# myfavouritekk/vdetlib

Measured on AMD Instinct MI355X. Metric: boxes/sec whole-node (NMS+temporal-conv+link), 300f×10k-box synth; mAP parity, higher is better.
Workload: dtype f32; 1 GPU; configs[1]+[2]: 1 video/GPU, 300 frames x 10000 boxes x 200 classes; per-(frame,class) NMS thresh 0.30 + temporal max-pool w=3 + 3-tap temporal convolution; greedy tubelets: 10 tracks/class (stop < 0.90), IoU-link >= 0.50, spatial max-pool IoU > 0.70 + completion + temporal max-pool; frames=300, boxes=10000, classes=200, scores=rand, parallelism=video-per-gpu x1, 4 distinct videos in flight per GPU

## Files before the change

### include/vdet_hip.h

```cpp
#ifndef VDET_HIP_H
#define VDET_HIP_H

#include <stdint.h>

#ifdef __cplusplus
extern "C" {
#endif

typedef struct vdet_ctx vdet_ctx;

typedef enum vdet_status {
    VDET_OK = 0,
    VDET_EINVAL = -1,
    VDET_ECAP = -2,
    VDET_EHIP = -3,
    VDET_EDIVZERO = -4,
    VDET_ENOMEM = -5,
    VDET_EINDEX = -6,
    VDET_EAGAIN = -7
} vdet_status;


int vdet_create(vdet_ctx **out, int device);
int vdet_destroy(vdet_ctx *ctx);
// ... 67 lines not shown
                        int class0, int use_score_thresh, float score_thresh, int topk, double nms_thresh,
                        float *d_dets, int32_t *d_sel_idx, int32_t *d_det_cnt, int32_t *d_keep, int32_t *d_keep_cnt);

int vdet_nms_volume_ordered(vdet_ctx *ctx, const float *d_boxes, const uint16_t *d_order, const int32_t *d_ncand,
                            int64_t F, int64_t B, int64_t C, double thresh, int32_t *d_keep_idx,
                            int32_t *d_keep_cnt, int64_t cap);

int vdet_video_batch(vdet_ctx *ctx, const float *d_boxes, const float *d_scores, const int64_t *h_frame_off,
                     int64_t V, int64_t B, int64_t C, double nms_thres, double thres, int max_tracks,
                     double link_thres, int max_frames, float *d_tracks, float *d_anchors, int32_t *d_ntracks,
                     int64_t cap, int32_t *d_keep_idx, int32_t *d_keep_cnt, double overlap_thres, int window,
                     double *d_det_score, double *d_pooled, float *d_boxes_out);

int vdet_volume_pass_batch(vdet_ctx *ctx, const float *d_scores, const int64_t *h_frame_off, int64_t V, int64_t B,
                           int64_t C, int window, float pad_max, const float *h_taps, float bias, float pad_conv,
                           float *d_out_max, float *d_out_conv, int use_score_thresh, float score_thresh);

int vdet_argsort_volume(vdet_ctx *ctx, const float *d_scores, int layout, int64_t F, int64_t B, int64_t C,
                        int use_score_thresh, float score_thresh, uint16_t *d_order, int32_t *d_ncand);

int vdet_temporal_maxpool_f32(vdet_ctx *ctx, const float *d_in, float *d_out, int64_t F, int64_t S,
                              int window, float pad);

int vdet_temporal_conv_f32(vdet_ctx *ctx, const float *d_in, float *d_out, int64_t F, int64_t S,
                           const float *h_taps, int K, float bias, float pad);

int vdet_temporal_maxpool_conv_f32(vdet_ctx *ctx, const float *d_in, float *d_out_max, float *d_out_conv, int64_t F,
                                   int64_t S, int window, float pad_max, const float *h_taps, float bias, float pad_conv);

int vdet_volume_pass(vdet_ctx *ctx, const float *d_scores, int64_t F, int64_t B, int64_t C, int window,
                     float pad_max, const float *h_taps, float bias, float pad_conv, float *d_out_max,
                     float *d_out_conv, int use_score_thresh, float score_thresh);

int vdet_track_volume(vdet_ctx *ctx, const float *d_boxes, const float *d_scores, int64_t F, int64_t B,
                      int64_t C, double nms_thres, double thres, int max_tracks, double link_thres,
                      int max_frames, float *d_tracks, float *d_anchors, int32_t *d_ntracks);

int vdet_nms_track_volume(vdet_ctx *ctx, const float *d_boxes, const float *d_scores, int64_t F, int64_t B,
                          int64_t C, double nms_thres, double thres, int max_tracks, double link_thres,
                          int max_frames, float *d_tracks, float *d_anchors, int32_t *d_ntracks, int64_t cap,
                          int32_t *d_keep_idx, int32_t *d_keep_cnt);

int vdet_rescore_tracks(vdet_ctx *ctx, const float *d_tracks, const int32_t *d_ntracks, const float *d_boxes,
                        const float *d_scores, int64_t F, int64_t B, int64_t C, int max_tracks,
                        double overlap_thres, int window, double *d_det_score, double *d_pooled,
                        float *d_boxes_out);

int vdet_eval_gt_upload(vdet_ctx *ctx, const int32_t *h_vid, const int64_t *h_frame, const int32_t *h_slot, const double *h_boxes,
                        int64_t G, const int64_t *h_vid_nf, int64_t NV, int K, double *d_gt_boxes, int32_t *d_gt_off,
                        int64_t *d_vid_meta);

int vdet_eval_match_tracks(vdet_ctx *ctx, const double *d_gt_boxes, const int32_t *d_gt_off, const int64_t *d_vid_meta, int K,
                           int rule, double iou_thr, int vid, int64_t F, int64_t C, int T, const float *d_boxes, int box_stride,
                           const void *d_scores, int scores_f64, const int32_t *d_ntracks, const int32_t *h_col_slot,
                           int32_t *d_st_slot, double *d_st_score, uint8_t *d_st_tp, int64_t st_len, int64_t st_cap,
                           int64_t *h_count);

int vdet_eval_match_tracks_batch(vdet_ctx *ctx, const double *d_gt_boxes, const int32_t *d_gt_off, const int64_t *d_vid_meta,
                                 int K, int rule, double iou_thr, const int32_t *h_vid, const int64_t *h_frame_off, int64_t V,
                                 int64_t C, int T, const float *d_boxes, int box_stride, const void *d_scores, int scores_f64,
                                 const int32_t *d_ntracks, const int32_t *h_col_slot, int32_t *d_st_slot, double *d_st_score,
                                 uint8_t *d_st_tp, int64_t st_len, int64_t st_cap, int64_t *h_count);

int vdet_eval_match_keep(vdet_ctx *ctx, const double *d_gt_boxes, const int32_t *d_gt_off, const int64_t *d_vid_meta, int K,
                         int rule, double iou_thr, int vid, const float *d_boxes, const float *d_scores, int layout, int64_t F,
                         int64_t B, int64_t C, const int32_t *d_keep_idx, const int32_t *d_keep_cnt, int64_t cap,
// ... 199 lines not shown
```

### vdetlib_amd/_lib.py

```python
import ctypes
import importlib.util
import os
import threading

_HERE = os.path.dirname(os.path.abspath(__file__))
LIB_PATH = os.path.join(_HERE, "libvdet_hip.so")

VDET_OK, VDET_EINVAL, VDET_ECAP, VDET_EHIP, VDET_EDIVZERO, VDET_ENOMEM, VDET_EINDEX, VDET_EAGAIN = 0, -1, -2, -3, -4, -5, -6, -7
LAYOUT_FBC, LAYOUT_FCB = 0, 1

_i64, _f64, _f32, _vp, _ci = ctypes.c_int64, ctypes.c_double, ctypes.c_float, ctypes.c_void_p, ctypes.c_int
SYMBOLS = {
    "vdet_create": (_ci, [ctypes.POINTER(_vp), _ci]),
    "vdet_destroy": (_ci, [_vp]),
    "vdet_set_stream": (_ci, [_vp, _vp]),
    "vdet_reset_stream": (_ci, [_vp]),
    "vdet_sync": (_ci, [_vp]),
    "vdet_last_error": (ctypes.c_char_p, [_vp]),
    "vdet_version": (ctypes.c_char_p, []),
    "vdet_last_timing_ms": (_ci, [_vp, _vp]),
    "vdet_last_launches": (_ci, [_vp, _vp]),
    "vdet_set_timing": (_ci, [_vp, _ci]),
    "vdet_query": (_ci, [_vp, _ci]),
    "vdet_set_cache": (_ci, [_vp, _ci]),
    "vdet_invalidate": (_ci, [_vp]),
    "vdet_set_async": (_ci, [_vp, _ci]),
    "vdet_nms_f32": (_ci, [_vp, _vp, _i64, _i64, _ci, _f64, _vp, _vp, ctypes.POINTER(_i64)]),
    "vdet_track_det_nms_f32": (_ci, [_vp, _vp, _i64, _i64, _vp, _i64, _i64, _f64, _vp, ctypes.POINTER(_i64)]),
    "vdet_track_det_nms_batch": (_ci, [_vp, _vp, _vp, _i64, _vp, _vp, _i64, _i64, _f64, _vp, _vp]),
    "vdet_iou_f64": (_ci, [_vp, _vp, _i64, _vp, _i64, _vp]),
    "vdet_svm_scores_f64": (_ci, [_vp, _vp, _i64, _i64, _vp, _vp, _i64, _vp]),
    "vdet_svm_scores_f32": (_ci, [_vp, _vp, _i64, _i64, _vp, _vp, _i64, _vp]),
    "vdet_spatial_maxpool_f64": (_ci, [_vp, _vp, _vp, _i64, _vp, _vp, _vp, _i64, _f64, _vp, _vp]),
    "vdet_series_completion_f64": (_ci, [_vp, _vp, _vp, _i64]),
    "vdet_series_maxpool_f64": (_ci, [_vp, _vp, _vp, _vp, _i64, _ci, _f64]),
    "vdet_series_interp_f64": (_ci, [_vp, _vp, _vp, _vp, _vp, _vp, _i64, _ci, _vp]),
    "vdet_threshold_topk": (_ci, [_vp, _vp, _ci, _i64, _i64, _ci, _ci, _f64, _ci, _vp, _vp]),
    "vdet_conv1d_f32": (_ci, [_vp, _vp, _ci, _ci, _vp, _vp, _ci, _ci, _ci, _vp]),
    "vdet_nms_volume": (_ci, [_vp, _vp, _vp, _ci, _i64, _i64, _i64, _f64, _ci, _f32, _vp, _vp, _i64]),
    "vdet_nms_volume_topk": (_ci, [_vp, _vp, _vp, _ci, _i64, _i64, _i64, _f64, _ci, _f32, _ci, _vp, _vp, _i64]),
    "vdet_det_nms_volume": (_ci, [_vp, _vp, _vp, _i64, _i64, _i64, _ci, _ci, _f32, _ci, _f64, _vp, _vp, _vp, _vp, _vp]),
    "vdet_nms_volume_ordered": (_ci, [_vp, _vp, _vp, _vp, _i64, _i64, _i64, _f64, _vp, _vp, _i64]),
    "vdet_argsort_volume": (_ci, [_vp, _vp, _ci, _i64, _i64, _i64, _ci, _f32, _vp, _vp]),
    "vdet_video_batch": (_ci, [_vp, _vp, _vp, _vp, _i64, _i64, _i64, _f64, _f64, _ci, _f64, _ci, _vp, _vp, _vp, _i64, _vp, _vp,
                               _f64, _ci, _vp, _vp, _vp]),
    "vdet_volume_pass_batch": (_ci, [_vp, _vp, _vp, _i64, _i64, _i64, _ci, _f32, _vp, _f32, _f32, _vp, _vp, _ci, _f32]),
    "vdet_volume_pass": (_ci, [_vp, _vp, _i64, _i64, _i64, _ci, _f32, _vp, _f32, _f32, _vp, _vp, _ci, _f32]),
    "vdet_track_volume": (_ci, [_vp, _vp, _vp, _i64, _i64, _i64, _f64, _f64, _ci, _f64, _ci, _vp, _vp, _vp]),
    "vdet_nms_track_volume": (_ci, [_vp, _vp, _vp, _i64, _i64, _i64, _f64, _f64, _ci, _f64, _ci, _vp, _vp, _vp,
                                    _i64, _vp, _vp]),
    "vdet_rescore_tracks": (_ci, [_vp, _vp, _vp, _vp, _vp, _i64, _i64, _i64, _ci, _f64, _ci, _vp, _vp, _vp]),
    "vdet_temporal_maxpool_f32": (_ci, [_vp, _vp, _vp, _i64, _i64, _ci, _f32]),
    "vdet_temporal_conv_f32": (_ci, [_vp, _vp, _vp, _i64, _i64, _vp, _ci, _f32, _f32]),
    "vdet_temporal_maxpool_conv_f32": (_ci, [_vp, _vp, _vp, _vp, _i64, _i64, _ci, _f32, _vp, _f32, _f32]),
    "vdet_eval_gt_upload": (_ci, [_vp, _vp, _vp, _vp, _vp, _i64, _vp, _i64, _ci, _vp, _vp, _vp]),
    "vdet_eval_match_tracks": (_ci, [_vp, _vp, _vp, _vp, _ci, _ci, _f64, _ci, _i64, _i64, _ci, _vp, _ci, _vp, _ci, _vp, _vp,
                                     _vp, _vp, _vp, _i64, _i64, ctypes.POINTER(_i64)]),
    "vdet_eval_match_tracks_batch": (_ci, [_vp, _vp, _vp, _vp, _ci, _ci, _f64, _vp, _vp, _i64, _i64, _ci, _vp, _ci, _vp, _ci, _vp,
                                           _vp, _vp, _vp, _vp, _i64, _i64, ctypes.POINTER(_i64)]),
# ... 130 lines not shown
        if rc == VDET_OK:
            return
        msg = self.error()
        if rc == VDET_EDIVZERO:
            raise ZeroDivisionError("float division")
        if rc in (VDET_EINVAL, VDET_ECAP):
            raise ValueError(msg or "invalid argument")
        if rc == VDET_ENOMEM:
            raise MemoryError(msg)
        if rc == VDET_EINDEX:
            raise IndexError(msg or "list index out of range")
        if rc == VDET_EAGAIN:
            raise RetryError(msg)
        raise RuntimeError("libvdet_hip: %s (rc=%d)" % (msg, rc))

    def set_stream(self, stream_ptr):
        self.check(self.lib.vdet_set_stream(self.h, _vp(stream_ptr or 0)))

    def reset_stream(self):
        self.check(self.lib.vdet_reset_stream(self.h))

    def sync(self):
        self.check(self.lib.vdet_sync(self.h))

    def set_cache(self, on):
        self.check(self.lib.vdet_set_cache(self.h, 1 if on else 0))

    def invalidate(self):
        self.check(self.lib.vdet_invalidate(self.h))

    def set_async(self, on):
        self.check(self.lib.vdet_set_async(self.h, 1 if on else 0))

    def query(self, what):
        return int(self.lib.vdet_query(self.h, int(what)))

    def set_timing(self, on):
        self.check(self.lib.vdet_set_timing(self.h, int(on)))

    def last_timing(self):
        ms = (ctypes.c_float * 16)()
        n = (ctypes.c_int * 16)()
        self.check(self.lib.vdet_last_timing_ms(self.h, ms))
        self.check(self.lib.vdet_last_launches(self.h, n))
        names = ["iou_bits", "adj_build", "sort", "walk", "temporal", "merge_sort", "iou_bits_general", "other",
                 "transpose_keys", "track_pick", "track_link", "track_suppress", "rescore_spatial", "rescore_series",
                 "sort_fallback", "track_loop"]
        return {k: (float(ms[i]), int(n[i])) for i, k in enumerate(names)}


def get_context(device=-1):
    with _lock:
        c = _ctxs.get(device)
        if c is None:
            c = Context(device)
            _ctxs[device] = c
        return c
```

### vdetlib_amd/csrc/temporal_kernels.hpp

```cpp
#pragma once
#include <hip/hip_runtime.h>
#include <stdint.h>

#include "nms_kernels.hpp"

namespace vdet {

struct Taps { float w[32]; };

__device__ __forceinline__ bool seg_in(const int2 *__restrict__ seg, int64_t f, int64_t g, int64_t F)
{
    if (!seg) return g >= 0 && g < F;
    const int2 r = seg[f];
    return g >= (int64_t)r.x && g < (int64_t)r.y;
}

__device__ __forceinline__ float4 splat4(float v) { return make_float4(v, v, v, v); }

struct MaxAcc {
    float4 m; uint32_t nan;
    __device__ __forceinline__ void init(float4 v)
    {
        m = v;
        nan = (v.x != v.x) | ((v.y != v.y) << 1) | ((v.z != v.z) << 2) | ((v.w != v.w) << 3);
// ... 224 lines not shown
            const float4 s = win[i][H];
            uint4 k4 = make_uint4(score_key(s.x), score_key(s.y), score_key(s.z), score_key(s.w));
            if (use_thr) {
                if (!(s.x > thr)) k4.x = 0u;
                if (!(s.y > thr)) k4.y = 0u;
                if (!(s.z > thr)) k4.z = 0u;
                if (!(s.w > thr)) k4.w = 0u;
            }
            tb[loff[i]] = k4.x; tb[loff[i] + TB] = k4.y; tb[loff[i] + 2 * TB] = k4.z; tb[loff[i] + 3 * TB] = k4.w;
        }
        __syncthreads();
        uint32_t *kf = keys + (int64_t)f * C4 * 4 * B + b0;
        const bool vec_ok = (B & 3) == 0;
#pragma unroll
        for (int i = 0; i < ITEMS; ++i) {
            const int idx = tid + NT * i;
            const int cc = idx >> (tb_shift - 2), q = idx & qmask;
            if (cc < C4 * 4 && 4 * q < rows) {
                const uint4 k4 = *reinterpret_cast<const uint4 *>(tb + cc * TB + ((4 * q) ^ (((cc >> 2) & qmask) << 2)));
                const int o = cc * B + 4 * q;
                if (vec_ok && 4 * q + 3 < rows) {
                    vp_store_u4(reinterpret_cast<uint4 *>(kf + o), k4);
                } else {
                    kf[o] = k4.x;
                    if (4 * q + 1 < rows) kf[o + 1] = k4.y;
                    if (4 * q + 2 < rows) kf[o + 2] = k4.z;
                    if (4 * q + 3 < rows) kf[o + 3] = k4.w;
                }
            }
        }
    }
}

template <int MODE>
__global__ __launch_bounds__(256) void temporal_scalar_kernel(const float *__restrict__ in, float *__restrict__ out,
                                                              int64_t F, int64_t S, int W, float pad, float bias,
                                                              Taps taps, const int2 *__restrict__ seg)
{
    const int64_t i = (int64_t)blockIdx.x * 256 + threadIdx.x;
    if (i >= F * S) return;
    const int64_t f = i / S, s = i - f * S;
    const int H = W / 2;
    if (MODE == 0) {
        float m = 0.0f;
        bool nan = false;
        for (int k = 0; k < W; ++k) {
            const int64_t g = f + k - H;
            const int64_t gc = min(max(g, (int64_t)0), F - 1);
            float v = in[gc * S + s];
            v = (g == gc && seg_in(seg, f, g, F)) ? v : pad;
            nan |= (v != v);
            m = (k == 0) ? v : fmaxf(m, v);
        }
        out[i] = nan ? __uint_as_float(0x7FC00000u) : m;
    } else {
        float acc = bias;
        for (int k = 0; k < W; ++k) {
            const int64_t g = f + k - H;
            const int64_t gc = min(max(g, (int64_t)0), F - 1);
            float v = in[gc * S + s];
            v = (g == gc && seg_in(seg, f, g, F)) ? v : pad;
            acc = acc + taps.w[k] * v;
        }
        out[i] = acc;
    }
}
// ... 30 lines not shown
```

### vdetlib_amd/csrc/vdet_capi.hip

```cpp
#include <hip/hip_runtime.h>
#include <atomic>
#include <chrono>

#include <algorithm>
#include <cmath>
#include <cstdarg>
#include <cstdio>
#include <cstdlib>
#include <cstring>
#include <string>
#include <vector>

#include "../../include/vdet_hip.h"
#include "nms_kernels.hpp"
#include "binsort_kernels.hpp"
#include "small_kernels.hpp"
#include "detnms_kernels.hpp"
#include "fused_kernels.hpp"
#include "adjrows_kernels.hpp"
#include "graphlists_kernels.hpp"
#include "temporal_kernels.hpp"
#include "tubelet_kernels.hpp"
#include "track_kernels.hpp"
#include "batch_kernels.hpp"
// ... 59 lines not shown
{
    if (cnt->pool_used > cnt->pool_max) cnt->pool_max = cnt->pool_used;
}

struct StagedTab {
    DevBuf dev;
    std::vector<char> host;
    std::vector<char> key;
    bool valid = false;
    long long uploads = 0;
};

struct ListsKey {
    const void *scores = nullptr;
    int64_t C = 0;
    int layout = -1, use_thr = 0;
    float thr = 0;
    int topk = 0;
    bool operator==(const ListsKey &o) const { return scores == o.scores && C == o.C && layout == o.layout && use_thr == o.use_thr && (!use_thr || thr == o.thr) && topk == o.topk; }
};

struct NmsPlan {
    std::vector<GroupDesc> groups;
    std::vector<TileDesc> tiles;
    std::vector<TilePair> pairs;
    std::vector<std::pair<int, int>> batch_tiles;
    std::vector<std::pair<int, int>> batch_pairs;
    std::vector<ListItem> ditems;
    std::vector<std::pair<int, int>> batch_ditems;
    size_t bits_words_max = 0;
    int64_t ntot = 0;
    int nmax = 0;
};

}

struct vdet_ctx {
    int device = 0;
    hipStream_t stream = nullptr;
    hipStream_t own_stream = nullptr;
    std::string err;
    Counters *d_cnt = nullptr;
    int latched = 0;
    size_t bits_budget = (size_t)1 << 30;
    size_t max_lds = 160 * 1024;
    int n_cu = 256;
    DevBuf boxes, scores, keys, excl, frames, groups, tiles, bits, rowz, rowmeta, groupz, adj, comp, origidx,
        out64, trk_frames, trk_boxes, b1, b2, iou_out, order, ncand, keepidx, keepcnt, gflags, pairs, tkeys, tstate, visited, heads, xkeys, xord, wmeta, wmeta16, reachtab, rowperm, qreach, ditems, striptot, stripoff, xncand, xbox, xbox16, xord16, xcum, xinfo, tmp[8];
    bool timing = false;
    bool timing_accumulate = false;
    std::vector<std::pair<hipEvent_t, hipEvent_t>> ev_pool;
    std::vector<int> ev_stage;
    size_t ev_used = 0;
    float last_ms[ST_COUNT] = {0};
    int last_launches[ST_COUNT] = {0};
    bool sort_attr_set = false;
    bool cache_enabled = false;
    struct PrepKey { const void *boxes = nullptr; int64_t F = 0, B = 0; float t32 = 0; ListsKey lists; } prep;
    bool graph_valid = false, lists_valid = false;
    struct KeySrc { const void *scores = nullptr; int64_t F = 0, B = 0, C = 0; int use_thr = 0; float thr = 0; } keysrc;
    bool keys_valid = false;
    bool vpass_attr_set = false;
    bool index_valid = false; const void *index_boxes = nullptr; int64_t index_F = 0, index_B = 0;
    bool all_regular = false;
    bool wave_transpose = false;
    bool no_lazy = false;
    bool no_index = false;
    bool force_general = false;
    bool atomic_rank = false;
    bool small_lists = true;
    bool adj_rows = true;
    bool direct_lists = true;
    uint32_t direct_cap = 384;
    int64_t direct_ntot = 0;
    unsigned long long direct_fixed = 0;
    bool no_fused = false;
    bool binsort = true;
    const std::vector<GroupDesc> *host_groups = nullptr;
    bool sym_built = false;
    NmsPlan vplan;
    bool vplan_valid = false;
    int64_t vplan_F = 0, vplan_B = 0;
    size_t vplan_budget = 0;
    long long n_host_syncs = 0;
    bool async_enabled = false;
    unsigned long long pool_hint = 0;
    bool topk_attr_set = false;
    float gt32 = 0.f;
    bool wmeta16_built = false;
    bool wmeta_built = false;
    bool last_sort_binned = false;
    StagedTab vidtab, segtab;
    DevBuf sortctl;
    DevBuf nover;
    DevBuf ordncand;
// ... 1139 lines not shown
    }
    if (device < 0) {
        if (hipGetDevice(&device) != hipSuccess) { delete c; return VDET_EHIP; }
    }
    if (device >= ndev || hipSetDevice(device) != hipSuccess) { delete c; return VDET_EINVAL; }
    c->device = device;
    hipDeviceProp_t prop;
    if (hipGetDeviceProperties(&prop, device) == hipSuccess) {
        c->n_cu = prop.multiProcessorCount > 0 ? prop.multiProcessorCount : 256;
        if (strncmp(prop.gcnArchName, "gfx950", 6) != 0) c->max_lds = 64 * 1024;
    }
    if (const char *e = getenv("VDET_FORCE_GENERAL")) c->force_general = atoi(e) != 0;
    if (const char *e = getenv("VDET_BITS_BUDGET_MB")) {
        const long mb = atol(e);
        if (mb > 0) c->bits_budget = (size_t)mb << 20;
    }
    if (hipStreamCreateWithFlags(&c->own_stream, hipStreamNonBlocking) != hipSuccess ||
        hipMalloc((void **)&c->d_cnt, sizeof(Counters)) != hipSuccess) {
        delete c;
        return VDET_EHIP;
    }
    c->stream = c->own_stream;
    (void)hipMemsetAsync(c->d_cnt, 0, sizeof(Counters), c->stream);
    if (const char *e = getenv("VDET_NO_INDEX")) c->no_index = atoi(e) != 0;
    if (const char *e = getenv("VDET_NO_LAZY")) c->no_lazy = atoi(e) != 0;
    if (const char *e = getenv("VDET_NO_FUSED")) c->no_fused = atoi(e) != 0;
    if (const char *e = getenv("VDET_ADJ_ROWS")) c->adj_rows = atoi(e) != 0;
    if (const char *e = getenv("VDET_DIRECT_LISTS")) c->direct_lists = atoi(e) != 0;
    if (const char *e = getenv("VDET_DIRECT_CAP")) { const int v = atoi(e); if (v >= 8 && v <= 32760) c->direct_cap = (uint32_t)(v & ~7); }
    if (const char *e = getenv("VDET_BINSORT")) c->binsort = atoi(e) != 0;
    if (const char *e = getenv("VDET_SMALL_LISTS")) c->small_lists = atoi(e) != 0;
    if (const char *e = getenv("VDET_TCN_TILED")) c->tcn_tiled = atoi(e) != 0;
    if (const char *e = getenv("VDET_TCN_GLOBAL")) c->tcn_global = atoi(e) != 0;
    {
        const int npat = 4096;
        std::vector<uint8_t> pats((size_t)npat * 64);
        uint32_t rs = 12345u;
        auto rnd = [&]() { rs = rs * 1664525u + 1013904223u; return rs >> 8; };
        for (int t = 0; t < npat; ++t) {
            const int kind = t % 8;
            const int nd = kind == 0 ? 1 : kind == 1 ? 2 : kind == 2 ? 3 : kind == 3 ? 8 : kind == 4 ? 32 : kind == 5 ? 64 : kind == 6 ? 200 : 254;
            for (int l = 0; l < 64; ++l) {
                uint8_t d = (uint8_t)(rnd() % nd);
                if (kind == 7 && (rnd() & 3) == 0) d = 255;
                if (t % 16 == 9) d = (uint8_t)((l * (1 + t % 7)) % nd);
                pats[(size_t)t * 64 + l] = d;
            }
        }
        bool ok = false;
        DevBuf pb;
        if (pb.reserve(pats.size()) == hipSuccess &&
            hipMemcpyAsync(pb.p, pats.data(), pats.size(), hipMemcpyHostToDevice, c->stream) == hipSuccess) {
            hipLaunchKernelGGL(lds_atomic_order_probe, dim3(256), dim3(64), 0, c->stream, pb.as<uint8_t>(), npat,
                               &c->d_cnt->status);
            Counters h;
            if (hipMemcpyAsync(&h, c->d_cnt, sizeof h, hipMemcpyDeviceToHost, c->stream) == hipSuccess &&
                host_sync(c) == hipSuccess)
                ok = (h.status == 0);
        }
        pb.release();
        (void)hipMemsetAsync(c->d_cnt, 0, sizeof(Counters), c->stream);
        c->atomic_rank = ok;
        if (const char *e = getenv("VDET_ATOMIC_RANK")) c->atomic_rank = c->atomic_rank && atoi(e) != 0;
    }
    {
        const int n = 64;
// ... 62 lines not shown
{
    if (!c) return VDET_EINVAL;
    c->stream = c->own_stream;
    return VDET_OK;
}

const char *vdet_last_error(vdet_ctx *c) { return c ? c->err.c_str() : "null context"; }

int vdet_set_cache(vdet_ctx *c, int enable)
{
    if (!c) return VDET_EINVAL;
    c->cache_enabled = enable != 0;
    c->graph_valid = c->lists_valid = c->index_valid = c->keys_valid = c->nodes_valid = false;
    return VDET_OK;
}

int vdet_invalidate(vdet_ctx *c)
{
    if (!c) return VDET_EINVAL;
    c->graph_valid = c->lists_valid = c->index_valid = c->keys_valid = c->nodes_valid = false;
    return VDET_OK;
}

int vdet_query(vdet_ctx *c, int what)
{
    if (!c) return VDET_EINVAL;
    if (what == 0) return c->atomic_rank ? 1 : 0;
    if (what == 1) return c->n_cu;
    if (what == 2) return c->all_regular ? 1 : 0;
    if (what == 3) return c->wave_transpose ? 1 : 0;
    if (what == 8) return (int)std::min<long long>(c->n_host_syncs, 0x7FFFFFFF);
    if (what == 10) return (int)std::min<long long>(c->tcn_params.uploads, 0x7FFFFFFF);
    if (what == 11) return (int)std::min<long long>(c->anchor_tab.uploads, 0x7FFFFFFF);
    if (what == 9) {
        if (!c->last_sort_binned || !c->sortctl.p) return -1;
        BinSortCtl h{};
        if (hipMemcpyAsync(&h, c->sortctl.p, sizeof h, hipMemcpyDeviceToHost, c->stream) != hipSuccess || host_sync(c) != hipSuccess) return VDET_EHIP;
        return h.nfail;
    }
    if (what >= 4 && what <= 7) {
        unsigned int h[4] = {0, 0, 0, 0};
        if (!c->linkstats.p) return 0;
        if (hipMemcpyAsync(h, c->linkstats.p, 16, hipMemcpyDeviceToHost, c->stream) != hipSuccess ||
            host_sync(c) != hipSuccess) return VDET_EHIP;
        return (int)std::min<unsigned int>(h[what - 4], 0x7FFFFFFFu);
    }
    return VDET_EINVAL;
}

int vdet_set_timing(vdet_ctx *c, int enable)
{
    if (!c) return VDET_EINVAL;
    c->timing = enable != 0;
    c->timing_accumulate = enable == 2;
    c->ev_used = 0;
    return VDET_OK;
}

int vdet_last_timing_ms(vdet_ctx *c, float *out16)
{
    float *out8 = out16;
    if (!c || !out8) return VDET_EINVAL;
    HIPCHK(c, host_sync(c));
    for (int i = 0; i < ST_COUNT; ++i) { c->last_ms[i] = 0; c->last_launches[i] = 0; }
    for (size_t i = 0; i < c->ev_used; ++i) {
        float ms = 0;
// ... 26 lines not shown
    c->latched = 0;
    if ((h.status & kStPoolAsync) || l == VDET_EAGAIN) {
        c->graph_valid = c->lists_valid = c->nodes_valid = false;
        if (h.status & kStDirect) {
            c->direct_lists = false;
            unsigned long long need = 0ull;
            if (c->direct_ntot > 0 && c->striptot.reserve(8) == hipSuccess &&
                hipMemsetAsync(c->striptot.p, 0, 8, c->stream) == hipSuccess) {
                hipLaunchKernelGGL(deg_sum_kernel, dim3(1024), dim3(256), 0, c->stream, c->rowz.as<uint32_t>(), c->direct_ntot,
                                   c->striptot.as<unsigned long long>());
                if (hipMemcpyAsync(&need, c->striptot.p, 8, hipMemcpyDeviceToHost, c->stream) != hipSuccess || host_sync(c) != hipSuccess) need = 0ull;
            }
            const unsigned long long dyn = h.pool_used > c->direct_fixed ? h.pool_used - c->direct_fixed : 0ull;
            h.pool_used = need + dyn + 4096;
            c->pool_hint = 0;
        }
        c->pool_hint = std::max(c->pool_hint, h.pool_used);
        if (h.pool_used <= 0xFFFFFFFFull) (void)c->adj.reserve((size_t)(h.pool_used + h.pool_used / 2) * 2 + 4096);
        if (l && l != VDET_EAGAIN) return l;
        return fail(c, VDET_EAGAIN, "adjacency pool overflow in an asynchronous graph build (%llu entries needed): the "
                                    "results since the last vdet_sync are invalid; the pool has been enlarged, run the calls again",
                    (unsigned long long)h.pool_used);
    }
    if (l) return l;
    c->pool_hint = std::max(c->pool_hint, h.pool_used);
    if (h.eindex) return fail(c, VDET_EINDEX, "list index out of range");
    return translate_status(c, h.status);
}

int vdet_set_async(vdet_ctx *c, int enable)
{
    if (!c) return VDET_EINVAL;
    c->async_enabled = enable != 0;
    return VDET_OK;
}

int vdet_nms_f32(vdet_ctx *c, const float *h_dets, int64_t n, int64_t ld, int ncols, double thresh,
                 const int64_t *h_order, int64_t *h_keep, int64_t *n_keep)
{
    if (!c || !n_keep) return VDET_EINVAL;
    *n_keep = 0;
    if (n < 0 || (ncols != 5 && ncols != 6) || (n > 0 && (!h_dets || !h_keep || ld < ncols)))
        return fail(c, VDET_EINVAL, "dets must be float32 [n,%d]", ncols);
    if (n == 0) return VDET_OK;
    if (n > 0x7FFFFFFF) return fail(c, VDET_EINVAL, "too many detections");
    HIPCHK(c, hipSetDevice(c->device));
    timing_reset(c);
    if (n <= kFusedMax && !c->no_fused)
        return fused_call(c, h_dets, n, ld, ncols, thresh, h_order, nullptr, 0, 0, h_keep, n_keep);
    const int o = ncols == 6 ? 1 : 0;

    NmsPlan pl;
    std::vector<int64_t> perm;
    if (o) {
        int rc = group_by_frame(c, h_dets, n, ld, perm, pl.groups);
        if (rc) return rc;
    } else {
        if (n > 32767) return fail(c, VDET_EINVAL, "%lld boxes in one image; the limit is 32767", (long long)n);
        perm.resize((size_t)n);
        for (int64_t i = 0; i < n; ++i) perm[(size_t)i] = i;
        pl.groups.push_back({0, (int32_t)n, 0});
    }
    make_plan(c, pl);

    std::vector<float> hb((size_t)n * 4), hs((size_t)n);
    std::vector<uint32_t> hidx((size_t)n), hkeys;
// ... 877 lines not shown
        int2 *seg = reinterpret_cast<int2 *>(dst);
        for (int64_t v = 0; v < V; ++v)
            for (int64_t f = h_frame_off[v]; f < h_frame_off[v + 1]; ++f) seg[f] = make_int2((int)h_frame_off[v], (int)h_frame_off[v + 1]);
    });
}

int vdet_volume_pass_batch(vdet_ctx *c, const float *d_scores, const int64_t *h_frame_off, int64_t V, int64_t B, int64_t C,
                           int window, float pad_max, const float *h_taps, float bias, float pad_conv, float *d_out_max,
                           float *d_out_conv, int use_score_thresh, float score_thresh)
{
    if (!c) return VDET_EINVAL;
    HIPCHK(c, hipSetDevice(c->device));
    int64_t F = 0;
    const int rc = upload_segments(c, h_frame_off, V, &F);
    if (rc) return rc;
    return volume_pass_impl(c, d_scores, F, B, C, window, pad_max, h_taps, bias, pad_conv, d_out_max, d_out_conv, use_score_thresh,
                            score_thresh, c->segtab.dev.as<int2>());
}

static int volume_pass_impl(vdet_ctx *c, const float *d_scores, int64_t F, int64_t B, int64_t C, int window, float pad_max,
                            const float *h_taps, float bias, float pad_conv, float *d_out_max, float *d_out_conv,
                            int use_score_thresh, float score_thresh, const int2 *d_seg)
{
    if (!c) return VDET_EINVAL;
    if (window < 1 || window % 2 != 1) return fail(c, VDET_EINVAL, "Window size must be odd!");
    if (window > 31) return fail(c, VDET_EINVAL, "taps: K must be odd and <= 31");
    if (F < 0 || B < 0 || C < 0 || F * B * C > ((int64_t)1 << 40)) return fail(c, VDET_EINVAL, "bad shape");
    if (F == 0 || B == 0 || C == 0) return VDET_OK;
    const bool conv = h_taps != nullptr;
    if (!d_scores || !d_out_max || (conv && !d_out_conv) || d_scores == d_out_max || (conv && (d_scores == d_out_conv || d_out_max == d_out_conv)))
        return fail(c, VDET_EINVAL, "bad volume_pass arguments");
    if (B > 32767 || F * C > 0x7FFFFFF0ll || F * B > 0x7FFFFFF0ll) return fail(c, VDET_EINVAL, "volume too large");
    c->keys_valid = false;
    const int64_t C4 = C / 4;
    int items = 0, TB = 0, NT = 0;
    if (C % 4 == 0 && (window == 3 || window == 5) &&
        (((uintptr_t)d_scores | (uintptr_t)d_out_max | (uintptr_t)(conv ? d_out_conv : d_out_max)) & 15) == 0) {
        for (int nt : {256, 512}) {
            int tb = 64;
            while (tb >= 16 && (int64_t)tb * C4 > (int64_t)nt * 4) tb >>= 1;
            if (tb >= 16 && (nt == 512 || tb >= 32)) { items = 4; TB = tb; NT = nt; break; }
        }
        if (items && (size_t)2 * C4 * TB * 16 > c->max_lds / 2) items = 0;
    }
    if (!items) {
        if (conv) return temporal_maxpool_conv_impl(c, d_scores, d_out_max, d_out_conv, F, B * C, window, pad_max, h_taps, bias, pad_conv, d_seg);
        Taps t0{};
        return temporal_launch(c, 0, d_scores, d_out_max, F, B * C, window, pad_max, 0.0f, t0, d_seg);
    }
    HIPCHK(c, hipSetDevice(c->device));
    timing_reset(c);
    if (!lists_match(c, ListsKey{d_scores, C, VDET_LAYOUT_FBC, use_score_thresh ? 1 : 0, score_thresh, 0}, F, B)) c->lists_valid = false;
    HIPCHK(c, c->tkeys.reserve((size_t)(F * C * B) * 4));
    Taps taps{};
    if (conv) for (int k = 0; k < window; ++k) taps.w[k] = h_taps[k];
    const int ntiles = (int)((B + TB - 1) / TB);
    int64_t chunks = std::min<int64_t>(std::max<int64_t>(F / 8, 1), (8 * c->n_cu + ntiles - 1) / ntiles);
    chunks = std::max<int64_t>(1, std::min<int64_t>(chunks, 65535));
    const int fchunk = (int)((F + chunks - 1) / chunks);
    const dim3 grid((unsigned)ntiles, (unsigned)((F + fchunk - 1) / fchunk));
    const size_t lds = (size_t)2 * C4 * TB * 16;
    int tb_shift = 0;
    while ((1 << tb_shift) < TB) ++tb_shift;
    const void *fn = nullptr;
#define VDET_VP(WW, CV, NTV) reinterpret_cast<const void *>(volume_pass_kernel<WW, 4, CV, NTV>)
    if (window == 3) fn = NT == 256 ? (conv ? VDET_VP(3, true, 256) : VDET_VP(3, false, 256)) : (conv ? VDET_VP(3, true, 512) : VDET_VP(3, false, 512));
    else fn = NT == 256 ? (conv ? VDET_VP(5, true, 256) : VDET_VP(5, false, 256)) : (conv ? VDET_VP(5, true, 512) : VDET_VP(5, false, 512));
    if (!c->vpass_attr_set) {
        for (const void *f : {VDET_VP(3, true, 256), VDET_VP(3, false, 256), VDET_VP(3, true, 512), VDET_VP(3, false, 512),
                              VDET_VP(5, true, 256), VDET_VP(5, false, 256), VDET_VP(5, true, 512), VDET_VP(5, false, 512)})
            HIPCHK(c, hipFuncSetAttribute(f, hipFuncAttributeMaxDynamicSharedMemorySize, (int)c->max_lds));
        c->vpass_attr_set = true;
    }
#undef VDET_VP
    const float4 *in4 = reinterpret_cast<const float4 *>(d_scores);
    float4 *om = reinterpret_cast<float4 *>(d_out_max), *oc = reinterpret_cast<float4 *>(d_out_conv);
    uint32_t *keys = c->tkeys.as<uint32_t>();
    int Fi = (int)F, Bi = (int)B, C4i = (int)C4;
    void *args[] = {&in4, &om, &oc, &keys, &Fi, &Bi, &C4i, &TB, &tb_shift, (void *)&fchunk, &pad_max, &pad_conv, &bias, &taps,
                    &use_score_thresh, &score_thresh, (void *)&d_seg};
    {
        StageTimer tm(c, ST_TEMPORAL);
        HIPCHK(c, hipLaunchKernel(fn, grid, dim3((unsigned)NT), args, lds, c->stream));
    }
    HIPCHK(c, hipGetLastError());
    c->keysrc.scores = d_scores; c->keysrc.F = F; c->keysrc.B = B; c->keysrc.C = C;
    c->keysrc.use_thr = use_score_thresh ? 1 : 0; c->keysrc.thr = score_thresh;
    c->keys_valid = true;
    return VDET_OK;
}

extern "C++" {
template <typename T>
static int svm_scores_impl(vdet_ctx *c, const T *h_feat, int64_t n, int64_t k, const T *h_W, const T *h_B, int64_t m, T *h_out)
{
    if (!c || n < 0 || k < 0 || m < 0) return VDET_EINVAL;
    if (n == 0 || m == 0) return VDET_OK;
    if ((k > 0 && (!h_feat || !h_W)) || !h_out) return fail(c, VDET_EINVAL, "null buffer");
    if (n * k > ((int64_t)1 << 34) || k * m > ((int64_t)1 << 34) || n * m > ((int64_t)1 << 34)) return fail(c, VDET_EINVAL, "matrix too large");
    HIPCHK(c, hipSetDevice(c->device));
    timing_reset(c);
    int rc;
    if ((rc = upload(c, c->tmp[0], h_feat, (size_t)(n * k) * sizeof(T)))) return rc;
    if ((rc = upload(c, c->tmp[1], h_W, (size_t)(k * m) * sizeof(T)))) return rc;
    if (h_B && (rc = upload(c, c->tmp[2], h_B, (size_t)m * sizeof(T)))) return rc;
    HIPCHK(c, c->tmp[3].reserve((size_t)(n * m) * sizeof(T)));
    {
        StageTimer tm(c, ST_OTHER);
        hipLaunchKernelGGL(svm_scores_kernel<T>, dim3((unsigned)((m + 63) / 64), (unsigned)((n + 63) / 64)), dim3(256), 0, c->stream,
                           c->tmp[0].as<T>(), c->tmp[1].as<T>(), h_B ? c->tmp[2].as<T>() : (const T *)nullptr, n, k, m, c->tmp[3].as<T>());
    }
    HIPCHK(c, hipGetLastError());
    HIPCHK(c, hipMemcpyAsync(h_out, c->tmp[3].p, (size_t)(n * m) * sizeof(T), hipMemcpyDeviceToHost, c->stream));
    HIPCHK(c, host_sync(c));
    return VDET_OK;
}
}

int vdet_svm_scores_f64(vdet_ctx *c, const double *h_feat, int64_t n, int64_t k, const double *h_W, const double *h_B, int64_t m,
                        double *h_out)
{
// ... 1603 lines not shown
```

Before: 334.4 million boxes/s.

## Add lean persistent volume-pass kernel and one-block-per-CU LDS occupancy mode

Adds a persistent 2-items-per-thread volume pass kernel with a grid of about 2×CUs and a waves_per_eu hint, selected only when the form is set to LEAN. It also adds a one-per-CU mode that inflates dynamic LDS so only one block fits per CU. That mode turns on by default when async and cache are enabled with window 3 and NT 512. The aim is to reduce cache and bandwidth contention from oversubscribed blocks while 4 videos are in flight, at the cost of less latency hiding from lower occupancy.

```diff
diff --git a/include/vdet_hip.h b/include/vdet_hip.h
--- a/include/vdet_hip.h
+++ b/include/vdet_hip.h
@@ -123,6 +123,12 @@
                      float pad_max, const float *h_taps, float bias, float pad_conv, float *d_out_max,
                      float *d_out_conv, int use_score_thresh, float score_thresh);
 
+#define VDET_VPASS_AUTO 0
+#define VDET_VPASS_CURRENT 1
+#define VDET_VPASS_LEAN 2
+#define VDET_VPASS_ONE_PER_CU 3
+int vdet_set_vpass(vdet_ctx *ctx, int form, int fchunk);
+
 int vdet_track_volume(vdet_ctx *ctx, const float *d_boxes, const float *d_scores, int64_t F, int64_t B,
                       int64_t C, double nms_thres, double thres, int max_tracks, double link_thres,
                       int max_frames, float *d_tracks, float *d_anchors, int32_t *d_ntracks);
diff --git a/vdetlib_amd/_lib.py b/vdetlib_amd/_lib.py
--- a/vdetlib_amd/_lib.py
+++ b/vdetlib_amd/_lib.py
@@ -25,6 +25,7 @@
     "vdet_set_cache": (_ci, [_vp, _ci]),
     "vdet_invalidate": (_ci, [_vp]),
     "vdet_set_async": (_ci, [_vp, _ci]),
+    "vdet_set_vpass": (_ci, [_vp, _ci, _ci]),
     "vdet_nms_f32": (_ci, [_vp, _vp, _i64, _i64, _ci, _f64, _vp, _vp, ctypes.POINTER(_i64)]),
     "vdet_track_det_nms_f32": (_ci, [_vp, _vp, _i64, _i64, _vp, _i64, _i64, _f64, _vp, ctypes.POINTER(_i64)]),
     "vdet_track_det_nms_batch": (_ci, [_vp, _vp, _vp, _i64, _vp, _vp, _i64, _i64, _f64, _vp, _vp]),
@@ -221,6 +222,9 @@
     def set_async(self, on):
         self.check(self.lib.vdet_set_async(self.h, 1 if on else 0))
 
+    def set_vpass(self, form=0, fchunk=0):
+        self.check(self.lib.vdet_set_vpass(self.h, int(form), int(fchunk)))
+
     def query(self, what):
         return int(self.lib.vdet_query(self.h, int(what)))
 
diff --git a/vdetlib_amd/csrc/temporal_kernels.hpp b/vdetlib_amd/csrc/temporal_kernels.hpp
--- a/vdetlib_amd/csrc/temporal_kernels.hpp
+++ b/vdetlib_amd/csrc/temporal_kernels.hpp
@@ -280,6 +280,140 @@
     }
 }
 
+template <int W, int ITEMS, bool CONV, int NT>
+__global__ __launch_bounds__(NT) __attribute__((amdgpu_waves_per_eu(8, 8)))
+void volume_pass_lean_kernel(const float4 *__restrict__ in, float4 *__restrict__ out_max, float4 *__restrict__ out_conv,
+                             uint32_t *__restrict__ keys, int F, int B, int C4, int TB, int tb_shift, int fchunk,
+                             float pad_max, float pad_conv, float bias, Taps taps, int use_thr, float thr,
+                             const int2 *__restrict__ seg)
+{
+    extern __shared__ __attribute__((aligned(16))) unsigned char vp_smem[];
+    uint32_t *tile = reinterpret_cast<uint32_t *>(vp_smem);
+    constexpr int H = W / 2;
+    const int tid = threadIdx.x;
+    const int ntiles = (B + TB - 1) / TB;
+    const int nwork = ntiles * ((F + fchunk - 1) / fchunk);
+    const int64_t S4 = (int64_t)B * C4;
+    const int tile_sz = C4 * 4 * TB;
+    const int qmask = (TB >> 2) - 1;
+    const bool vec_ok = (B & 3) == 0;
+    const float4 pm = splat4(pad_max), pc = splat4(pad_conv);
+    for (int w = blockIdx.x; w < nwork; w += gridDim.x) {
+        const int wy = w / ntiles;
+        const int b0 = (w - wy * ntiles) * TB;
+        const int rows = min(TB, B - b0);
+        const int n4 = rows * C4;
+        const int f0 = wy * fchunk;
+        const int f1 = min(F, f0 + fchunk);
+        const char *in_t = reinterpret_cast<const char *>(in + (int64_t)b0 * C4);
+        char *om_t = reinterpret_cast<char *>(out_max + (int64_t)b0 * C4);
+        char *oc_t = CONV ? reinterpret_cast<char *>(out_conv + (int64_t)b0 * C4) : nullptr;
+        uint32_t goff[ITEMS];
+        int loff[ITEMS];
+        bool on[ITEMS];
+#pragma unroll
+        for (int i = 0; i < ITEMS; ++i) {
+            const int idx = tid + NT * i;
+            on[i] = idx < n4;
+            const int idc = min(idx, n4 - 1);
+            const int b = idc / C4, c4 = idc - b * C4;
+            goff[i] = (uint32_t)idc * 16u;
+            loff[i] = 4 * c4 * TB + (b ^ ((c4 & qmask) << 2));
+        }
+        float4 win[ITEMS][W];
+        float4 nxt[ITEMS];
+        bool ok[W];
+#pragma unroll
+        for (int k = 0; k < W - 1; ++k) {
+            const int g = f0 - H + k;
+            const int gc = min(max(g, 0), F - 1);
+            const char *fin = in_t + (int64_t)gc * S4 * 16;
+#pragma unroll
+            for (int i = 0; i < ITEMS; ++i) win[i][k + 1] = *reinterpret_cast<const float4 *>(fin + goff[i]);
+            ok[k + 1] = (g == gc);
+        }
+        {
+            const char *fin = in_t + (int64_t)min(f0 + H, F - 1) * S4 * 16;
+#pragma unroll
+            for (int i = 0; i < ITEMS; ++i) nxt[i] = *reinterpret_cast<const float4 *>(fin + goff[i]);
+        }
+        if (w != (int)blockIdx.x) __syncthreads();
+        for (int f = f0; f < f1; ++f) {
+#pragma unroll
+            for (int k = 0; k < W - 1; ++k) {
+                ok[k] = ok[k + 1];
+#pragma unroll
+                for (int i = 0; i < ITEMS; ++i) win[i][k] = win[i][k + 1];
+            }
+            ok[W - 1] = (f + H <= F - 1);
+            if (seg) {
+#pragma unroll
+                for (int k = 0; k < W; ++k) ok[k] = seg_in(seg, f, f - H + k, F);
+            }
+#pragma unroll
+            for (int i = 0; i < ITEMS; ++i) win[i][W - 1] = nxt[i];
+            {
+                const char *fin = in_t + (int64_t)min(f + 1 + H, F - 1) * S4 * 16;
+#pragma unroll
+                for (int i = 0; i < ITEMS; ++i) nxt[i] = *reinterpret_cast<const float4 *>(fin + goff[i]);
+            }
+            uint32_t *tb = tile + (f & 1) * tile_sz;
+            char *om = om_t + (int64_t)f * S4 * 16;
+            char *oc = CONV ? oc_t + (int64_t)f * S4 * 16 : nullptr;
+#pragma unroll
+            for (int i = 0; i < ITEMS; ++i) {
+                if (!on[i]) continue;
+                MaxAcc a;
+                a.init(ok[0] ? win[i][0] : pm);
+#pragma unroll
+                for (int k = 1; k < W; ++k) a.add(ok[k] ? win[i][k] : pm);
+                vp_store(reinterpret_cast<float4 *>(om + goff[i]), a.get());
+                if (CONV) {
+                    float4 r = splat4(bias);
+#pragma unroll
+                    for (int k = 0; k < W; ++k) {
+                        const float t = taps.w[k];
+                        const float4 v = ok[k] ? win[i][k] : pc;
+                        r.x = r.x + t * v.x; r.y = r.y + t * v.y;
+                        r.z = r.z + t * v.z; r.w = r.w + t * v.w;
+                    }
+                    vp_store(reinterpret_cast<float4 *>(oc + goff[i]), r);
+                }
+                const float4 s = win[i][H];
+                uint4 k4 = make_uint4(score_key(s.x), score_key(s.y), score_key(s.z), score_key(s.w));
+                if (use_thr) {
+                    if (!(s.x > thr)) k4.x = 0u;
+                    if (!(s.y > thr)) k4.y = 0u;
+                    if (!(s.z > thr)) k4.z = 0u;
+                    if (!(s.w > thr)) k4.w = 0u;
+                }
+                tb[loff[i]] = k4.x; tb[loff[i] + TB] = k4.y; tb[loff[i] + 2 * TB] = k4.z; tb[loff[i] + 3 * TB] = k4.w;
+            }
+            __syncthreads();
+            char *kf = reinterpret_cast<char *>(keys + (int64_t)f * C4 * 4 * B + b0);
+            int ct = tid;
+            asm volatile("" : "+v"(ct));
+#pragma unroll
+            for (int i = 0; i < ITEMS; ++i) {
+                const int idx = ct + NT * i;
+                const int cc = idx >> (tb_shift - 2), q = idx & qmask;
+                if (cc < C4 * 4 && 4 * q < rows) {
+                    const uint4 k4 = *reinterpret_cast<const uint4 *>(tb + cc * TB + ((4 * q) ^ (((cc >> 2) & qmask) << 2)));
+                    uint32_t *ko = reinterpret_cast<uint32_t *>(kf + (uint32_t)(cc * B + 4 * q) * 4u);
+                    if (vec_ok && 4 * q + 3 < rows) {
+                        vp_store_u4(reinterpret_cast<uint4 *>(ko), k4);
+                    } else {
+                        ko[0] = k4.x;
+                        if (4 * q + 1 < rows) ko[1] = k4.y;
+                        if (4 * q + 2 < rows) ko[2] = k4.z;
+                        if (4 * q + 3 < rows) ko[3] = k4.w;
+                    }
+                }
+            }
+        }
+    }
+}
+
 template <int MODE>
 __global__ __launch_bounds__(256) void temporal_scalar_kernel(const float *__restrict__ in, float *__restrict__ out,
                                                               int64_t F, int64_t S, int W, float pad, float bias,
diff --git a/vdetlib_amd/csrc/vdet_capi.hip b/vdetlib_amd/csrc/vdet_capi.hip
--- a/vdetlib_amd/csrc/vdet_capi.hip
+++ b/vdetlib_amd/csrc/vdet_capi.hip
@@ -115,6 +115,7 @@
     int64_t ntot = 0;
     int nmax = 0;
 };
+
 
 }
 
@@ -144,6 +145,9 @@
     struct KeySrc { const void *scores = nullptr; int64_t F = 0, B = 0, C = 0; int use_thr = 0; float thr = 0; } keysrc;
     bool keys_valid = false;
     bool vpass_attr_set = false;
+    int vpass_form = VDET_VPASS_AUTO;
+    int vpass_fchunk = 0;
+    int vpass_last_items = 0;
     bool index_valid = false; const void *index_boxes = nullptr; int64_t index_F = 0, index_B = 0;
     bool all_regular = false;
     bool wave_transpose = false;
@@ -1349,6 +1353,8 @@
     if (const char *e = getenv("VDET_SMALL_LISTS")) c->small_lists = atoi(e) != 0;
     if (const char *e = getenv("VDET_TCN_TILED")) c->tcn_tiled = atoi(e) != 0;
     if (const char *e = getenv("VDET_TCN_GLOBAL")) c->tcn_global = atoi(e) != 0;
+    if (const char *e = getenv("VDET_VPASS_FORM")) { const int v = atoi(e); if (v >= VDET_VPASS_AUTO && v <= VDET_VPASS_ONE_PER_CU) c->vpass_form = v; }
+    if (const char *e = getenv("VDET_VPASS_FCHUNK")) { const int v = atoi(e); if (v >= 1) c->vpass_fchunk = v; }
     {
         const int npat = 4096;
         std::vector<uint8_t> pats((size_t)npat * 64);
@@ -1477,6 +1483,7 @@
     if (what == 8) return (int)std::min<long long>(c->n_host_syncs, 0x7FFFFFFF);
     if (what == 10) return (int)std::min<long long>(c->tcn_params.uploads, 0x7FFFFFFF);
     if (what == 11) return (int)std::min<long long>(c->anchor_tab.uploads, 0x7FFFFFFF);
+    if (what == 12) return c->vpass_last_items;
     if (what == 9) {
         if (!c->last_sort_binned || !c->sortctl.p) return -1;
         BinSortCtl h{};
@@ -1569,6 +1576,15 @@
 {
     if (!c) return VDET_EINVAL;
     c->async_enabled = enable != 0;
+    return VDET_OK;
+}
+
+int vdet_set_vpass(vdet_ctx *c, int form, int fchunk)
+{
+    if (!c) return VDET_EINVAL;
+    if (form < VDET_VPASS_AUTO || form > VDET_VPASS_ONE_PER_CU || fchunk < 0) return fail(c, VDET_EINVAL, "bad volume pass form");
+    c->vpass_form = form;
+    c->vpass_fchunk = fchunk;
     return VDET_OK;
 }
 
@@ -2512,17 +2528,28 @@
         return fail(c, VDET_EINVAL, "bad volume_pass arguments");
     if (B > 32767 || F * C > 0x7FFFFFF0ll || F * B > 0x7FFFFFF0ll) return fail(c, VDET_EINVAL, "volume too large");
     c->keys_valid = false;
+    c->vpass_last_items = 0;
     const int64_t C4 = C / 4;
     int items = 0, TB = 0, NT = 0;
+    const int form = c->vpass_form;
     if (C % 4 == 0 && (window == 3 || window == 5) &&
         (((uintptr_t)d_scores | (uintptr_t)d_out_max | (uintptr_t)(conv ? d_out_conv : d_out_max)) & 15) == 0) {
-        for (int nt : {256, 512}) {
+        if (window == 3 && form == VDET_VPASS_LEAN) {
             int tb = 64;
-            while (tb >= 16 && (int64_t)tb * C4 > (int64_t)nt * 4) tb >>= 1;
-            if (tb >= 16 && (nt == 512 || tb >= 32)) { items = 4; TB = tb; NT = nt; break; }
+            while (tb >= 16 && (int64_t)tb * C4 > 512 * 2) tb >>= 1;
+            if (tb >= 16) { items = 2; TB = tb; NT = 512; }
+        }
+        if (!items) {
+            for (int nt : {256, 512}) {
+                int tb = 64;
+                while (tb >= 16 && (int64_t)tb * C4 > (int64_t)nt * 4) tb >>= 1;
+                if (tb >= 16 && (nt == 512 || tb >= 32)) { items = 4; TB = tb; NT = nt; break; }
+            }
         }
         if (items && (size_t)2 * C4 * TB * 16 > c->max_lds / 2) items = 0;
     }
+    const bool one_per_cu = items == 4 && (form == VDET_VPASS_ONE_PER_CU ||
+                                           (form == VDET_VPASS_AUTO && c->async_enabled && c->cache_enabled && window == 3 && NT == 512));
     if (!items) {
         if (conv) return temporal_maxpool_conv_impl(c, d_scores, d_out_max, d_out_conv, F, B * C, window, pad_max, h_taps, bias, pad_conv, d_seg);
         Taps t0{};
@@ -2537,21 +2564,29 @@
     const int ntiles = (int)((B + TB - 1) / TB);
     int64_t chunks = std::min<int64_t>(std::max<int64_t>(F / 8, 1), (8 * c->n_cu + ntiles - 1) / ntiles);
     chunks = std::max<int64_t>(1, std::min<int64_t>(chunks, 65535));
-    const int fchunk = (int)((F + chunks - 1) / chunks);
-    const dim3 grid((unsigned)ntiles, (unsigned)((F + fchunk - 1) / fchunk));
-    const size_t lds = (size_t)2 * C4 * TB * 16;
+    const int fchunk = c->vpass_fchunk > 0 ? (int)std::min<int64_t>(std::max<int64_t>(c->vpass_fchunk, (F + 65534) / 65535), F)
+                                           : (int)((F + chunks - 1) / chunks);
+    const int64_t nchunks = (F + fchunk - 1) / fchunk;
+    const dim3 grid = items == 2 ? dim3((unsigned)std::min<int64_t>(nchunks * ntiles, 2 * (int64_t)c->n_cu))
+                                 : dim3((unsigned)ntiles, (unsigned)nchunks);
+    size_t lds = (size_t)2 * C4 * TB * 16;
+    if (one_per_cu) lds = std::max(lds, c->max_lds / 2 + 16);
     int tb_shift = 0;
     while ((1 << tb_shift) < TB) ++tb_shift;
     const void *fn = nullptr;
 #define VDET_VP(WW, CV, NTV) reinterpret_cast<const void *>(volume_pass_kernel<WW, 4, CV, NTV>)
-    if (window == 3) fn = NT == 256 ? (conv ? VDET_VP(3, true, 256) : VDET_VP(3, false, 256)) : (conv ? VDET_VP(3, true, 512) : VDET_VP(3, false, 512));
+#define VDET_VPL(CV) reinterpret_cast<const void *>(volume_pass_lean_kernel<3, 2, CV, 512>)
+    if (items == 2) fn = conv ? VDET_VPL(true) : VDET_VPL(false);
+    else if (window == 3) fn = NT == 256 ? (conv ? VDET_VP(3, true, 256) : VDET_VP(3, false, 256)) : (conv ? VDET_VP(3, true, 512) : VDET_VP(3, false, 512));
     else fn = NT == 256 ? (conv ? VDET_VP(5, true, 256) : VDET_VP(5, false, 256)) : (conv ? VDET_VP(5, true, 512) : VDET_VP(5, false, 512));
     if (!c->vpass_attr_set) {
         for (const void *f : {VDET_VP(3, true, 256), VDET_VP(3, false, 256), VDET_VP(3, true, 512), VDET_VP(3, false, 512),
-                              VDET_VP(5, true, 256), VDET_VP(5, false, 256), VDET_VP(5, true, 512), VDET_VP(5, false, 512)})
+                              VDET_VP(5, true, 256), VDET_VP(5, false, 256), VDET_VP(5, true, 512), VDET_VP(5, false, 512),
+                              VDET_VPL(true), VDET_VPL(false)})
             HIPCHK(c, hipFuncSetAttribute(f, hipFuncAttributeMaxDynamicSharedMemorySize, (int)c->max_lds));
         c->vpass_attr_set = true;
     }
+#undef VDET_VPL
 #undef VDET_VP
     const float4 *in4 = reinterpret_cast<const float4 *>(d_scores);
     float4 *om = reinterpret_cast<float4 *>(d_out_max), *oc = reinterpret_cast<float4 *>(d_out_conv);
@@ -2567,6 +2602,7 @@
     c->keysrc.scores = d_scores; c->keysrc.F = F; c->keysrc.B = B; c->keysrc.C = C;
     c->keysrc.use_thr = use_score_thresh ? 1 : 0; c->keysrc.thr = score_thresh;
     c->keys_valid = true;
+    c->vpass_last_items = items + (one_per_cu ? 100 : 0);
     return VDET_OK;
 }
 
```

Result: faster. 346.9 million boxes/s (median of 6 runs) (+3.7%).
